# yuanzhi-zhu/DiffPIR

Hardware: AMD Instinct MI355X
Metric: restored images/sec @100 NFE, 256x256 (higher is better)
Workload: dtype f32 (GEMMs as 3 x f16 MFMA on hi/lo-split fp32 operands, fp32 accumulate; exact-fp32-MFMA mode in alt_precision); 1 GPU; configs[1]: ffhq topology 256x256 deblur (61x61 Gaussian PSF), 100 NFE, batch 16/GPU, device Philox noise, hipGraph=on; global_batch=16, nfe=100, collective=none

## Files before the change

diffpir_amd/_lib.py:

```python
from __future__ import annotations

import ctypes as C
import os

_HERE = os.path.dirname(os.path.abspath(__file__))
LIB_PATH = os.environ.get("DIFFPIR_LIB") or os.path.join(_HERE, "csrc", "libdiffpir_hip.so")
ABI_VERSION = 2



class UNetDesc(C.Structure):
    _fields_ = [("image_size", C.c_int32), ("in_channels", C.c_int32), ("model_channels", C.c_int32),
                ("out_channels", C.c_int32), ("num_res_blocks", C.c_int32), ("num_head_channels", C.c_int32),
                ("n_channel_mult", C.c_int32), ("channel_mult", C.c_float * 8),
                ("n_attention_ds", C.c_int32), ("attention_ds", C.c_int32 * 8), ("num_classes", C.c_int32)]


class Tensor(C.Structure):
    _fields_ = [("name", C.c_char_p), ("data", C.c_void_p), ("ndim", C.c_int32), ("shape", C.c_int64 * 4)]


class Step(C.Structure):
    _fields_ = [("t", C.c_int32), ("last", C.c_int32), ("c1", C.c_float), ("c2", C.c_float), ("tau", C.c_float),
                ("sa_t", C.c_float), ("s1m_t", C.c_float), ("sa_p", C.c_float),
# ... 160 lines not shown
    "dpir_unet_flops": (C.c_double, [C.c_void_p, C.c_int, C.c_int]),
    "dpir_unet_flops_class": (C.c_double, [C.c_void_p, C.c_int, C.c_int, C.c_int]),
}

_lib = None


class EngineLibraryError(RuntimeError):
    pass


DEBUG_LIB_PATH = os.path.join(_HERE, "csrc", "libdiffpir_dbg.so")
_dbg = None


def load_debug():
    global _dbg
    if _dbg is not None:
        return _dbg
    load()
    if not os.path.exists(DEBUG_LIB_PATH):
        raise EngineLibraryError(f"{DEBUG_LIB_PATH} not found: `make -C diffpir_amd/csrc` builds it next to the product library")
    d = C.CDLL(DEBUG_LIB_PATH)
    d.dpir_debug_conv_bench.argtypes = [C.c_void_p] + [C.c_int] * 10 + [C.POINTER(C.c_double)]
    d.dpir_debug_conv7_emit_supported.argtypes = [C.c_void_p] + [C.c_int] * 4 + [C.POINTER(C.c_int)]
    d.dpir_debug_victim.argtypes = [C.c_void_p, C.c_int, C.c_int, C.c_int, C.c_longlong, C.c_int, C.POINTER(C.c_ulonglong)]
    d.dpir_debug_victim_alu.argtypes = [C.c_void_p, C.c_int, C.c_int, C.c_int, C.c_int, C.POINTER(C.c_ulonglong)]
    for fn in (d.dpir_debug_victim_fft_pk, d.dpir_debug_victim_fft_nopk):
        fn.argtypes = [C.c_void_p, C.c_int, C.c_int, C.c_int, C.POINTER(C.c_ulonglong)]
    d.dpir_debug_conv7_check.argtypes = [C.c_void_p] + [C.c_int] * 10 + [C.POINTER(C.c_double), C.POINTER(C.c_double), C.POINTER(C.c_ulonglong),
                                                                        C.POINTER(C.c_float), C.POINTER(C.c_int)]
    d.dpir_debug_conv5_layer.argtypes = [C.c_void_p] + [C.c_int] * 7 + [C.c_void_p] * 7 + [C.POINTER(C.c_int)]
    d.dpir_debug_conv5_layer.restype = C.c_int
    d.dpir_debug_conv3_layer.argtypes = [C.c_void_p, C.POINTER(Conv3Desc)]
    d.dpir_debug_conv3_layer.restype = C.c_int
    d.dpir_debug_conv9_layer.argtypes = [C.c_void_p, C.POINTER(Conv9Desc)]
    d.dpir_debug_conv9_layer.restype = C.c_int
    d.dpir_debug_conv11_layer.argtypes = [C.c_void_p, C.POINTER(Conv11Desc)]
    d.dpir_debug_conv11_layer.restype = C.c_int
    d.dpir_debug_conv11_counts.argtypes = [C.POINTER(C.c_longlong), C.POINTER(C.c_longlong)]
    d.dpir_debug_conv11_counts.restype = None
    d.dpir_debug_conv_up_layer.argtypes = [C.c_void_p, C.POINTER(ConvUpDesc)]
    d.dpir_debug_conv_up_layer.restype = C.c_int
    d.dpir_debug_conv_up_counts.argtypes = [C.POINTER(C.c_longlong), C.POINTER(C.c_longlong)]
    d.dpir_debug_conv_up_counts.restype = None
    d.dpir_debug_attention.argtypes = [C.c_void_p, C.POINTER(AttentionDesc)]
    d.dpir_debug_attention.restype = C.c_int
    d.dpir_debug_groupnorm.argtypes = [C.c_void_p, C.POINTER(GroupNormDesc)]
    d.dpir_debug_groupnorm.restype = C.c_int
    for n in ("dpir_debug_conv_bench", "dpir_debug_victim", "dpir_debug_victim_alu", "dpir_debug_victim_fft_pk", "dpir_debug_victim_fft_nopk",
              "dpir_debug_conv7_check"):
        getattr(d, n).restype = C.c_int
    _dbg = d
    return d


def load():
    global _lib
    if _lib is not None:
        return _lib
    if not os.path.exists(LIB_PATH):
        raise EngineLibraryError(
            f"{LIB_PATH} not found: build it with `python -c 'import __graft_entry__ as g; g.build()'` "
            f"or `make -C diffpir_amd/csrc`.  There is no CPU fallback.")
    try:
        import torch
# ... 18 lines not shown
```

diffpir_amd/csrc/dbg_conv.hip:

```cpp
#include "engine.h"
#include "conv6_params.h"
#include "conv9.h"
#include "conv11.h"
#include "conv_up.h"
#include "../../include/diffpir_debug.h"
#include <string.h>
#include <vector>
using namespace dpir;
static int fail(dpir_engine* e, const Status& s) {
    if (e) e->last_error = s.msg;
    return s.code;
}
#define API_TRY(e, expr)                          \
    do {                                          \
        Status _s = (expr);                       \
        if (!_s.ok()) return fail((e), _s);       \
    } while (0)
#define API_HIP(e, expr)                                                                  \
    do {                                                                                  \
        hipError_t _h = (expr);                                                           \
        if (_h != hipSuccess)                                                             \
            return fail((e), Status{DPIR_ERR_HIP, std::string(#expr) + ": " + hipGetErrorString(_h)}); \
    } while (0)

__global__ void dbg_bitdiff_kernel(const float* a, const float* b, size_t n, unsigned long long* out) {
    unsigned long long cnt = 0; unsigned mx = 0;
    for (size_t i = (size_t)blockIdx.x * blockDim.x + threadIdx.x; i < n; i += (size_t)gridDim.x * blockDim.x) {
        const float x = a[i], y = b[i];
        if (__builtin_bit_cast(unsigned, x) != __builtin_bit_cast(unsigned, y)) {
            ++cnt;
            const float d = fabsf(x - y);
            const unsigned u = d == d ? __builtin_bit_cast(unsigned, d) : 0x7fc00000u;
            mx = u > mx ? u : mx;
        }
    }
    if (cnt) { atomicAdd(&out[0], cnt); atomicMax(&out[1], (unsigned long long)mx); }
}
// ... 149 lines not shown
    PendingConv pend;
    API_TRY(e, launch_conv6(e->stream, a6, &k6, &pend));
    if ((S > 1) != (k6 == 3) || (S > 1 && pend.ksplit != S)) return fail(e, Status{DPIR_ERR_INVALID, "conv7 check: the split rule of launch_conv6 changed"});
    API_TRY(e, launch_conv7(e->stream, k, blocks * S, x1 != 0));
    API_HIP(e, hipGetLastError());
    if (S > 1) {
        hipLaunchKernelGGL(dbg_bitdiff_kernel, dim3(2048), dim3(256), 0, e->stream, p6, p7, (size_t)S * no, cmp);
    } else {
        hipLaunchKernelGGL(dbg_bitdiff_kernel, dim3(2048), dim3(256), 0, e->stream, o6, o7, no, cmp);
        hipLaunchKernelGGL(dbg_bitdiff_kernel, dim3(256), dim3(256), 0, e->stream, reinterpret_cast<const float*>(st6), reinterpret_cast<const float*>(st7), nst * 2, cmp);
    }
    unsigned long long h[2] = {0, 0};
    API_HIP(e, hipMemcpyAsync(h, cmp, 16, hipMemcpyDeviceToHost, e->stream));
    API_HIP(e, hipStreamSynchronize(e->stream));
    *mismatches_out = h[0];
    const unsigned mb = (unsigned)h[1];
    *maxdiff_out = __builtin_bit_cast(float, mb);
    hipEvent_t e0, e1, e2;
    API_HIP(e, hipEventCreate(&e0)); API_HIP(e, hipEventCreate(&e1)); API_HIP(e, hipEventCreate(&e2));
    for (int i = 0; i < 3; ++i) { API_TRY(e, launch_conv6(e->stream, a6, &k6, &pend)); API_TRY(e, launch_conv7(e->stream, k, blocks * S, x1 != 0)); }
    API_HIP(e, hipEventRecord(e0, e->stream));
    for (int i = 0; i < iters; ++i) API_TRY(e, launch_conv6(e->stream, a6, &k6, &pend));
    API_HIP(e, hipEventRecord(e1, e->stream));
    for (int i = 0; i < iters; ++i) API_TRY(e, launch_conv7(e->stream, k, blocks * S, x1 != 0));
    API_HIP(e, hipEventRecord(e2, e->stream));
    API_HIP(e, hipEventSynchronize(e2));
    float m6 = 0, m7 = 0;
    API_HIP(e, hipEventElapsedTime(&m6, e0, e1)); API_HIP(e, hipEventElapsedTime(&m7, e1, e2));
    (void)hipEventDestroy(e0); (void)hipEventDestroy(e1); (void)hipEventDestroy(e2);
    *ms6_out = m6 / iters; *ms7_out = m7 / iters;
    return DPIR_OK;
}

int dpir_debug_conv5_layer(dpir_engine* e, int B, int ca, int cb, int Cout, int H, int W, int tile, const float* xa, const float* xb,
                           const float* w, const float* bias, const float* prm, const float* res, float* out, int* path_out) {
    if (!e || !xa || !w || !bias || !out || !path_out || B <= 0 || ca <= 0 || cb < 0 || (cb > 0 && !xb) || Cout <= 0 || tile < 0 || tile > 2) return DPIR_ERR_INVALID;
    if (e->precision == 0) return fail(e, invalid("conv5 layer: the engine is in f32 mode"));
    (void)hipSetDevice(e->device);
    const int C = ca + cb, HW = H * W;
    const size_t na = (size_t)B * ca * HW, nb = (size_t)B * cb * HW, no = (size_t)B * Cout * HW;
    float *dxa = nullptr, *dxb = nullptr, *dbias = nullptr, *dout = nullptr, *dres = nullptr, *dw = nullptr, *partial = nullptr; float4* dprm = nullptr;
    API_TRY(e, e->ws.getT("c5#xa", na, &dxa));
    API_TRY(e, e->ws.getT("c5#xb", nb + 1, &dxb));
    API_TRY(e, e->ws.getT("c5#b", (size_t)round_up(Cout, 64), &dbias));
    API_TRY(e, e->ws.getT("c5#o", no, &dout));
    API_TRY(e, e->ws.getT("c5#res", no, &dres));
    API_TRY(e, e->ws.getT("c5#prm", (size_t)B * C, &dprm));
    API_HIP(e, hipMemcpy(dxa, xa, na * 4, hipMemcpyHostToDevice));
    if (cb) API_HIP(e, hipMemcpy(dxb, xb, nb * 4, hipMemcpyHostToDevice));
    API_HIP(e, hipMemset(dbias, 0, (size_t)round_up(Cout, 64) * 4));
    API_HIP(e, hipMemcpy(dbias, bias, (size_t)Cout * 4, hipMemcpyHostToDevice));
    if (prm) API_HIP(e, hipMemcpy(dprm, prm, (size_t)B * C * 16, hipMemcpyHostToDevice));
    if (res) API_HIP(e, hipMemcpy(dres, res, no * 4, hipMemcpyHostToDevice));
    API_HIP(e, hipMemset(dout, 0xFF, no * 4));
    std::vector<uint16_t> w16v;
    const float w16_scale = pack_weights_f16x3_1x1(w, Cout, C, w16v);
    void* wp = nullptr;
    API_TRY(e, e->ws.get("c5#w16", w16v.size() * 2, &wp));
    API_HIP(e, hipMemcpy(wp, w16v.data(), w16v.size() * 2, hipMemcpyHostToDevice));
    const bool has_prm = prm != nullptr;
    const bool use5 = !(has_prm && C % 16) && (tile != 0 || conv5_supported(B, Cout, H, W, has_prm) || conv5_small_supported(B, ca, cb, Cout, H, W, has_prm));
    Status st;
    if (use5) {
        Conv5Args a5;
        a5.src = CatSrc{dxa, ca, cb ? dxb : nullptr, cb}; a5.prm = has_prm ? dprm : nullptr; a5.w16 = wp; a5.w16_scale = w16_scale;
        a5.bias = dbias; a5.out = dout; a5.res = res ? dres : nullptr; a5.B = B; a5.Cout = Cout; a5.H = H; a5.W = W;
        a5.x1 = e->precision == 2; a5.force_tile = tile;
        *path_out = tile ? tile : (conv5_small_supported(B, ca, cb, Cout, H, W, has_prm) ? 2 : 1);
        st = launch_conv5(e->stream, a5);
    } else {
        const int coutp = round_up(Cout, 64), cinp = round_up(C, 16);
        std::vector<float> packed((size_t)cinp * coutp, 0.f);
        for (int co = 0; co < Cout; ++co)
            for (int ci = 0; ci < C; ++ci) packed[(size_t)ci * coutp + co] = w[(size_t)co * C + ci];
        API_TRY(e, e->ws.getT("c5#w", packed.size(), &dw));
        API_HIP(e, hipMemcpy(dw, packed.data(), packed.size() * 4, hipMemcpyHostToDevice));
        API_TRY(e, e->ws.getT("conv#partial", (size_t)16 * 1024 * 1024, &partial));
        ConvArgs a;
        a.src.a = dxa; a.src.ca = ca; a.src.b = cb ? dxb : nullptr; a.src.cb = cb; a.src.Hs = H; a.src.Ws = W; a.src.mode = 0;
        a.src.prm = has_prm ? dprm : nullptr;
        a.w = dw; a.bias = dbias; a.out = dout; a.res = res ? dres : nullptr; a.res_mode = 0;
        a.B = B; a.Cin = C; a.Cout = Cout; a.CoutP = coutp; a.H = H; a.W = W; a.ks = 1;
        a.partial = partial; a.partial_capacity = (size_t)16 * 1024 * 1024;
        *path_out = 0;
        st = launch_conv(e->stream, a);
    }
    API_TRY(e, st);
    API_HIP(e, hipStreamSynchronize(e->stream));
    API_HIP(e, hipMemcpy(out, dout, no * 4, hipMemcpyDeviceToHost));
    return DPIR_OK;
}

int dpir_debug_conv3_layer(dpir_engine* e, dpir_debug_conv3_desc* d) {
    if (!e || !d) return DPIR_ERR_INVALID;
    d->path_out = -1; d->ksplit_out = 0; d->stat_kind_out = 0;
    const int B = d->B, ca = d->ca, cb = d->cb, Cout = d->Cout, H = d->H, W = d->W, mode = d->mode, C = ca + cb;
    if (!d->xa || !d->w || !d->bias || !d->out || B <= 0 || ca <= 0 || cb < 0 || (cb > 0 && !d->xb) || Cout <= 0 || H <= 0 || W <= 0 || mode < 0 || mode > 2 ||
        d->res_mode < -1 || d->res_mode > 2 || (d->res_mode >= 0 && !d->res) || d->prologue < 0 || d->prologue > 2 ||
        (d->route != 0 && d->route != 6 && d->route != 7 && d->route != 8))
        return fail(e, invalid("conv3 layer: bad descriptor"));
    if (d->prologue == 1 && !d->prm) return fail(e, invalid("conv3 layer: prologue 1 needs the table"));
    if (d->prologue == 2 && (!d->gamma || !d->beta)) return fail(e, invalid("conv3 layer: prologue 2 needs gamma and beta"));
    if (mode == 1 && ((H | W) & 1)) return fail(e, invalid("conv3 layer: a nearest-up source needs an even output size"));
    if (d->res_mode == 1 && ((H | W) & 1)) return fail(e, invalid("conv3 layer: a half-resolution residual needs an even output size"));
    if (d->defer && (!d->split || (d->route != 0 && d->route != 7) || !d->gamma2 || !d->beta2 || !d->w2 || !d->bias2 || !d->out2 || d->Cout2 <= 0))
        return fail(e, invalid("conv3 layer: defer needs split, route 0 or 7 and the second stage's operands"));
    (void)hipSetDevice(e->device);
    const int Hs = mode == 1 ? H / 2 : (mode == 2 ? H * 2 : H), Ws = mode == 1 ? W / 2 : (mode == 2 ? W * 2 : W);
    const size_t HWs = (size_t)Hs * Ws, HW = (size_t)H * W;
    const size_t na = (size_t)B * ca * HWs, nb = (size_t)B * cb * HWs, no = (size_t)B * Cout * HW;
    const size_t nres = d->res_mode == 1 ? no / 4 : (d->res_mode == 2 ? no * 4 : no);
    const int coutp = round_up(Cout, 64);
    float *dxa = nullptr, *dxb = nullptr, *dbias = nullptr, *dout = nullptr, *dres = nullptr, *scale = nullptr; float4* dprm = nullptr;
    API_TRY(e, e->ws.getT("c3#xa", na, &dxa));
    API_TRY(e, e->ws.getT("c3#xb", nb + 1, &dxb));
    API_TRY(e, e->ws.getT("c3#b", (size_t)coutp, &dbias));
    API_TRY(e, e->ws.getT("c3#o", no, &dout));
    API_TRY(e, e->ws.getT("c3#res", nres, &dres));
    API_TRY(e, e->ws.getT("c3#prm", (size_t)B * C, &dprm));
    API_TRY(e, e->ws.getT("c3#scale", (size_t)4, &scale));
    API_HIP(e, hipMemcpy(dxa, d->xa, na * 4, hipMemcpyHostToDevice));
    if (cb) API_HIP(e, hipMemcpy(dxb, d->xb, nb * 4, hipMemcpyHostToDevice));
    API_HIP(e, hipMemset(dbias, 0, (size_t)coutp * 4));
    API_HIP(e, hipMemcpy(dbias, d->bias, (size_t)Cout * 4, hipMemcpyHostToDevice));
// ... 569 lines not shown
```

diffpir_amd/csrc/unet.hip:

```cpp
#include "engine.h"
#include "conv6_params.h"
#include "conv9.h"
#include "conv11.h"
#include "conv_up.h"
#include <unordered_map>
#include <cstdint>
#include <math.h>
#include <string.h>
#include <stdlib.h>

namespace dpir {

Status Workspace::get(const std::string& name, size_t bytes, void** out) {
    auto it = bufs.find(name);
    if (it != bufs.end() && it->second.bytes >= bytes) { *out = it->second.p; return Status{}; }
    if (frozen) return Status{DPIR_ERR_STATE, "workspace allocation of '" + name + "' during graph capture"};
    if (it != bufs.end()) { (void)hipFree(it->second.p); total -= it->second.bytes; bufs.erase(it); }
    void* p = nullptr;
    size_t rb = (bytes + 255) & ~(size_t)255;
    hipError_t err = hipMalloc(&p, rb);
    if (err != hipSuccess) return Status{DPIR_ERR_NOMEM, "hipMalloc(" + std::to_string(rb) + ") for '" + name + "' failed"};
    bufs[name] = DevBuf{p, rb};
    total += rb;
    ++generation;
    *out = p;
    return Status{};
}
void Workspace::release() {
    for (auto& kv : bufs) (void)hipFree(kv.second.p);
    bufs.clear();
    total = 0;
}

namespace {
struct WeightMap {
    std::map<std::string, const dpir_tensor*> m;
// ... 322 lines not shown
                DPIR_TRY(ws.getT(tag + "#gst", (size_t)B * 32, &ga.stats_out));
                if (prm_out) *prm_out = ga.prm_out;
                if (stats_out) *stats_out = ga.stats_out;
            }
            {
                ProfScope ps(&e->prof, PC_ELEM);
                DPIR_TRY(launch_gn_act_small(s, ga));
            }
            if (pending.partial) { fused.erase(pending.out); pending = PendingConv{}; }
            return conv6_on_planes(cw, s16, plane, res, res_mode, out, Ho, Wo, emit);
        }
        DPIR_TRY(resolve());
        float4* prm = nullptr;
        DPIR_TRY(gn(g, in, tag, film_off, true, &prm, stats_out));
        if (prm_out) *prm_out = prm;
        return conv(cw, in, mode, prm, res, res_mode, out, Ho, Wo, emit);
    }

    bool conv9_route(const ConvW& cw, int Ho, int Wo, bool hop) const {
        static const bool on = !(getenv("DPIR_CONV9") && atoi(getenv("DPIR_CONV9")) == 0);
        static const int min_wg = getenv("DPIR_CONV9_MIN_WG") ? atoi(getenv("DPIR_CONV9_MIN_WG")) : kConv9MinWg;
        return on && !grad && e->precision != 0 && cw.w16 && cw.ks == 3 && conv9_supported(B, cw.cin, cw.cout, Ho, Wo, hop) &&
               (long long)B * (cw.cout / 32) >= min_wg;
    }

    bool conv11_route(const ConvW& cw, int Ho, int Wo, bool hop) const {
        static const bool on = !(getenv("DPIR_CONV11") && atoi(getenv("DPIR_CONV11")) == 0);
        static const int split_below = getenv("DPIR_SPLIT_BELOW") ? atoi(getenv("DPIR_SPLIT_BELOW")) : 256;
        if (!on || grad || e->precision != 1 || !cw.w11 || cw.ks != 3 || !conv11_supported(cw.cin, cw.cout, Ho, Wo)) return false;
        const long long wgs = (long long)(Wo / 32) * (Ho / 8) * B * (cw.cout / 128);
        return hop ? wgs >= 384 && conv11_emit_supported(cw.cout, Ho, Wo) : wgs >= split_below;
    }

    Status conv6_on_planes(const ConvW& cw, char* s16, size_t plane, const float* res, int res_mode, float* out, int Ho, int Wo,
                           const Conv6Emit* emit = nullptr) {
        const bool x1 = e->precision == 2;
        Conv6Args a6;
        a6.x1 = x1;
        a6.xhi = s16; a6.xlo = s16 + plane; a6.w16 = cw.w16; a6.w16_scale = cw.w16_scale;
        a6.bias = cw.bias; a6.out = out; a6.res = res; a6.res_mode = res_mode;
        a6.B = B; a6.Cin = cw.cin; a6.Cout = cw.cout; a6.H = Ho; a6.W = Wo;
        a6.partial = partial; a6.partial_capacity = partial_cap;
        const int slots = conv6_stat_slots(Ho, Wo);
        float2* st = nullptr; double2* sp = nullptr;
        if (slots > 0 && cw.cout % 32 == 0) {
            const std::string key = std::to_string(reinterpret_cast<uintptr_t>(out));
            DPIR_TRY(ws.getT("st#" + key, (size_t)B * cw.cout * slots, &st));
            DPIR_TRY(ws.getT("sp#" + key, (size_t)B * cw.cout, &sp));
        }
        a6.stat = st; a6.stat_plane = sp;
        a6.emit = emit;
        if (emit) { a6.stat = nullptr; a6.stat_plane = nullptr; a6.partial = nullptr; a6.partial_capacity = 0; }
        int kind = 0;
        PendingConv pc;
        ProfScope ps(&e->prof, PC_CONV3);
        if (conv9_route(cw, Ho, Wo, emit != nullptr)) {
            Conv9Args a9;
            a9.xhi = s16; a9.xlo = s16 + plane; a9.w16 = cw.w16; a9.w16_scale = cw.w16_scale; a9.bias = cw.bias; a9.out = out;
            a9.res = res; a9.res_mode = res_mode; a9.B = B; a9.Cin = cw.cin; a9.Cout = cw.cout; a9.H = Ho; a9.W = Wo;
            a9.stat_plane = emit ? nullptr : sp; a9.x1 = x1; a9.emit = emit;
            DPIR_TRY(launch_conv9(s, a9));
            if (sp && !emit) fused[out] = FusedStat{nullptr, 0, sp};
            else fused.erase(out);
            return Status{};
        }
        if (conv11_route(cw, Ho, Wo, emit != nullptr)) {
// ... 23 lines not shown
        if (pending.partial && (is_pending(in.a) || is_pending(in.b) || is_pending(res) || !use5)) DPIR_TRY(resolve());
        static const bool use_conv8 = !(getenv("DPIR_CONV8") && atoi(getenv("DPIR_CONV8")) == 0);
        if (use_conv8 && cw.w8 && prm && !grad && !emit && !res && mode == 0 && !in.b && in.H == Ho && in.W == Wo &&
            conv8_supported(B, in.C(), cw.cout, Ho, Wo)) {
            Conv8Args a8;
            a8.x = in.a; a8.prm = prm; a8.w = cw.w8; a8.w_scale = cw.w8_scale; a8.bias = cw.bias; a8.out = out;
            a8.B = B; a8.C = in.C(); a8.Cout = cw.cout; a8.H = Ho; a8.W = Wo; a8.range_ctr = e->range_ctr; a8.x1 = x1;
            fused.erase(out);
            ProfScope ps(&e->prof, PC_CONV3);
            return launch_conv8(s, a8);
        }
        if (cw.w16 && cw.ks == 3 && conv6_supported(Ho, Wo)) {
            int eh = mode == 1 ? Ho / 2 : (mode == 2 ? Ho * 2 : Ho), ew = mode == 1 ? Wo / 2 : (mode == 2 ? Wo * 2 : Wo);
            if (eh != in.H || ew != in.W) return invalid("conv: source resolution does not match mode");
            const int C = in.C(), C8 = 2 * ((C + 15) / 16);
            const size_t plane = (size_t)B * C8 * Ho * Wo * 16;
            if (plane >= ((size_t)1 << 32)) return invalid("conv: split activation plane exceeds the 4 GiB buffer-descriptor range; reduce the batch");
            char* s16 = nullptr;
            DPIR_TRY(ws.getT("act#s16", 2 * plane, &s16));
            {
                ProfScope ps(&e->prof, PC_ELEM);
                DPIR_TRY(launch_act_split(s, CatSrc{in.a, in.ca, in.b, in.cb}, prm, mode, B, Ho, Wo, s16, x1 ? nullptr : s16 + plane, e->range_ctr));
            }
            return conv6_on_planes(cw, s16, plane, res, res_mode, out, Ho, Wo, emit);
        }
        if (emit) return invalid("conv: fused emission was requested for a launch that is not on the f16 3x3 path");
        if (use5) {
            Conv5Args a5;
            a5.src = CatSrc{in.a, in.ca, in.b, in.cb}; a5.prm = prm; a5.w16 = cw.w16; a5.w16_scale = cw.w16_scale;
            a5.bias = cw.bias; a5.out = out; a5.res = res; a5.B = B; a5.Cout = cw.cout; a5.H = Ho; a5.W = Wo;
            a5.range_ctr = e->range_ctr; a5.x1 = x1;
            fused.erase(out);
            ProfScope ps(&e->prof, PC_CONV1);
            return launch_conv5(s, a5);
        }
        fused.erase(out);
        ConvArgs a;
        a.src.a = in.a; a.src.ca = in.ca; a.src.b = in.b; a.src.cb = in.cb; a.src.Hs = in.H; a.src.Ws = in.W;
        a.src.mode = mode; a.src.prm = prm;
        a.w = cw.w; a.bias = cw.bias; a.out = out; a.res = res; a.res_mode = res_mode;
        a.B = B; a.Cin = cw.cin; a.Cout = cw.cout; a.CoutP = cw.coutp; a.H = Ho; a.W = Wo; a.ks = cw.ks;
        a.partial = partial; a.partial_capacity = partial_cap;
        ProfScope ps(&e->prof, cw.ks == 3 ? PC_CONV3 : PC_CONV1);
        return launch_conv(s, a);
    }
    Status gn(const GnW& g, const Act& in, const std::string& tag, int film_off, bool silu, float4** prm_out, float2** stats_out = nullptr) {
        float4* prm = nullptr;
        float2* gst = nullptr;
        if (grad) DPIR_TRY(ws.getT(tag + "#gst", (size_t)B * 32, &gst));
        if (is_pending(in.a) || is_pending(in.b)) DPIR_TRY(resolve());
        DPIR_TRY(ws.getT(tag + "#prm", (size_t)B * g.c, &prm));
        GnStatSrc src[2];
        const float* tp[2] = {in.a, in.b};
        const int tc[2] = {in.ca, in.cb};
        for (int k = 0; k < 2; ++k) {
            src[k].c = tc[k];
            if (!tp[k] || tc[k] == 0) { src[k].c = 0; continue; }
            auto it = fused.find(tp[k]);
            if (it != fused.end()) { src[k].slots = it->second.slots; src[k].nslots = it->second.nslots; src[k].part = it->second.part; continue; }
            double2* part = nullptr;
            DPIR_TRY(ws.getT(tag + "#stats" + std::to_string(k), (size_t)B * tc[k], &part));
            ProfScope ps(&e->prof, PC_GN);
            DPIR_TRY(launch_gn_stats(s, CatSrc{tp[k], tc[k], nullptr, 0}, B, in.H * in.W, part));
            src[k].part = part;
        }
        ProfScope ps(&e->prof, PC_ELEM);
// ... 385 lines not shown
```

include/diffpir_debug.h:

```cpp
#ifndef DIFFPIR_DEBUG_H
#define DIFFPIR_DEBUG_H
#include "diffpir_engine.h"
#ifdef __cplusplus
extern "C" {
#endif
int dpir_debug_conv_bench(dpir_engine* e, int B, int Cin, int Cout, int H, int W, int ks, int mode, int with_prm,
                          int dbg, int iters, double* ms_out);
int dpir_debug_victim(dpir_engine* e, int lds_bytes, int threads, int blocks, long long spin_ticks, int iters, unsigned long long* bad_out);
int dpir_debug_victim_alu(dpir_engine* e, int mode, int blocks, int iters_in_kernel, int launches, unsigned long long* bad_out);
int dpir_debug_victim_fft_pk(dpir_engine* e, int blocks, int iters_in_kernel, int launches, unsigned long long* bad_out);
int dpir_debug_victim_fft_nopk(dpir_engine* e, int blocks, int iters_in_kernel, int launches, unsigned long long* bad_out);
int dpir_debug_conv7_check(dpir_engine* e, int B, int Cin, int Cout, int H, int W, int res_mode, int x1, int split, int scaled, int iters,
                           double* ms6_out, double* ms7_out, unsigned long long* mismatches_out, float* maxdiff_out, int* ksplit_out);
int dpir_debug_conv7_emit_supported(dpir_engine* e, int B, int Cout, int H, int W, int* capacity_out);
int dpir_debug_conv5_layer(dpir_engine* e, int B, int ca, int cb, int Cout, int H, int W, int tile, const float* xa, const float* xb,
                           const float* w, const float* bias, const float* prm, const float* res, float* out, int* path_out);
typedef struct dpir_debug_conv3_desc {
    int32_t B, ca, cb, Cout, H, W, mode, res_mode, scaled, prologue, route, split, defer, Cout2;
    const float *xa, *xb, *w, *bias, *res, *prm, *gamma, *beta, *film, *gamma2, *beta2, *w2, *bias2;
    float* out; double* stat_out; float* out2;
    int32_t stat_kind_out, path_out, ksplit_out, reserved;
} dpir_debug_conv3_desc;
int dpir_debug_conv3_layer(dpir_engine* e, dpir_debug_conv3_desc* d);
typedef struct dpir_debug_conv9_desc {
    int32_t B, Cin, Cout, H, W, res_mode, hop, Cout2;
    const float *x, *w, *bias, *res, *prm, *gamma2, *beta2, *film2, *w2, *bias2;
    float* out; double* stat_out; float* out2;
    int32_t ran_out, iters;
    double ms_out;
} dpir_debug_conv9_desc;
int dpir_debug_conv9_layer(dpir_engine* e, dpir_debug_conv9_desc* d);
typedef struct dpir_debug_conv11_desc {
    int32_t B, Cin, Cout, H, W, res_mode, route, ksplit, hop, Cout2;
    const float *x, *w, *bias, *res, *prm, *gamma2, *beta2, *film2, *w2, *bias2;
    float* out; double* stat_out; float* out2;
    int32_t ran_out, iters;
    double ms_out;
} dpir_debug_conv11_desc;
int dpir_debug_conv11_layer(dpir_engine* e, dpir_debug_conv11_desc* d);
void dpir_debug_conv11_counts(long long* plain, long long* hop);
typedef struct dpir_debug_conv_up_desc {
    int32_t B, Cin, Cout, Hs, Ws, hop, force_hop, Cout2, route, reserved;
    const float *x, *w, *bias, *res, *prm, *gamma2, *beta2, *film2, *w2, *bias2;
    float* out; double* stat_out; float* out2;
    int32_t ran_out, iters;
    double ms_out;
} dpir_debug_conv_up_desc;
int dpir_debug_conv_up_layer(dpir_engine* e, dpir_debug_conv_up_desc* d);
void dpir_debug_conv_up_counts(long long* plain, long long* hop);
// ... 20 lines not shown
```

Baseline: 9.565 images/s.

## Add K-split 1x1 conv kernel with per-wave channel chunks for deep low-pixel layers

Adds a new 1x1 convolution kernel for the f16-split MFMA path. Each of the four waves in a workgroup takes a strided subset of 16-channel input chunks, streams them through a per-wave LDS ring with DMA loads and register-held weights, then sums the partial accumulators through LDS in the epilogue. In the UNet it replaces launch_conv5 for layers with at least 32 input chunks whose grid fits within two resident workgroups per CU, targeting deep, low-resolution 1x1 convs that otherwise underfill the GPU. The cost is an extra LDS reduction and another code path; it can be disabled with an environment variable, and debug timing hooks are added.

```diff
diff --git a/diffpir_amd/_lib.py b/diffpir_amd/_lib.py
--- a/diffpir_amd/_lib.py
+++ b/diffpir_amd/_lib.py
@@ -216,6 +216,10 @@
                                                                         C.POINTER(C.c_float), C.POINTER(C.c_int)]
     d.dpir_debug_conv5_layer.argtypes = [C.c_void_p] + [C.c_int] * 7 + [C.c_void_p] * 7 + [C.POINTER(C.c_int)]
     d.dpir_debug_conv5_layer.restype = C.c_int
+    d.dpir_debug_conv5_layer_time.argtypes = [C.c_void_p] + [C.c_int] * 7 + [C.c_void_p] * 7 + [C.POINTER(C.c_int), C.c_int, C.POINTER(C.c_double)]
+    d.dpir_debug_conv5_layer_time.restype = C.c_int
+    d.dpir_debug_conv5k_count.argtypes = []
+    d.dpir_debug_conv5k_count.restype = C.c_longlong
     d.dpir_debug_conv3_layer.argtypes = [C.c_void_p, C.POINTER(Conv3Desc)]
     d.dpir_debug_conv3_layer.restype = C.c_int
     d.dpir_debug_conv9_layer.argtypes = [C.c_void_p, C.POINTER(Conv9Desc)]
diff --git a/diffpir_amd/csrc/conv5k.h b/diffpir_amd/csrc/conv5k.h
--- /dev/null
+++ b/diffpir_amd/csrc/conv5k.h
@@ -0,0 +1,12 @@
+#pragma once
+#include "common.h"
+namespace dpir {
+
+const char* conv5k_refusal(int B, int ca, int cb, int Cout, int H, int W, bool has_prm);
+Status launch_conv5k(hipStream_t s, const Conv5Args& a);
+long long conv5k_workgroups(int B, int Cout, int H, int W);
+int conv5k_resident_workgroups();
+constexpr int kConv5kMinChunks = 32;
+long long conv5k_launch_count();
+
+}
diff --git a/diffpir_amd/csrc/conv5k.hip b/diffpir_amd/csrc/conv5k.hip
--- /dev/null
+++ b/diffpir_amd/csrc/conv5k.hip
@@ -0,0 +1,340 @@
+#include "common.h"
+#include "lds_dma.h"
+#include "conv5k.h"
+#include <type_traits>
+#include <atomic>
+
+namespace dpir {
+
+typedef float floatx16 __attribute__((ext_vector_type(16)));
+typedef _Float16 half8 __attribute__((ext_vector_type(8)));
+
+struct Conv5kK {
+    const float* sa; const float* sb; int ca, cb;
+    unsigned bytes_a, bytes_b, bytes_w, bytes_prm;
+    const float4* prm;
+    const char* w16; const float* bias; float* out; const float* res;
+    int B, Cout, HW;
+    int n_chunks, n_co_blocks;
+    int n_wblocks;
+    int n_tiles, pair_xcd;
+    int total_px;
+    float out_scale;
+    unsigned long long* range_ctr;
+};
+
+template <int I, int N, class F>
+__device__ __forceinline__ void static_for5k(F&& f) {
+    if constexpr (I < N) {
+        f(std::integral_constant<int, I>{});
+        static_for5k<I + 1, N>(f);
+    }
+}
+
+__device__ __forceinline__ float gn_apply5k(float v, const float4 m, bool silu) {
+    float t = (v - m.x) * m.y + m.z;
+    if (silu) t = t * __builtin_amdgcn_rcpf(1.0f + __builtin_amdgcn_exp2f(t * -1.4426950408889634f));
+    return t;
+}
+
+typedef unsigned u32x4k __attribute__((ext_vector_type(4)));
+template <int IMM>
+__device__ __forceinline__ half8 load_a5k(unsigned voff, u32x4k rsrc, unsigned soff) {
+    half8 r;
+    asm volatile("buffer_load_dwordx4 %0, %1, %2, %3 offen offset:%4" : "=v"(r) : "v"(voff), "s"(rsrc), "s"(soff), "n"(IMM) : "memory");
+    return r;
+}
+
+constexpr int kC5kTpx = 128;
+constexpr int kC5kRedStride = kC5kTpx + 4;
+constexpr int kC5kRedBytes = 4 * 32 * kC5kRedStride * 4;
+static_assert(2 * (kC5kRedBytes + 256) <= 160 * 1024, "two workgroups per CU");
+
+template <bool HAS_PRM, bool X1>
+__device__ __forceinline__ bool conv5k_chunk(const float* __restrict__ xs, const float4* __restrict__ ps, const int (&pimg)[4], int l31, bool silu,
+                                             const half8 (&ah)[2], const half8 (&al)[2], floatx16 (&acc)[2][4]) {
+    bool bad = false;
+#pragma unroll
+    for (int jp = 0; jp < 4; jp += 2) {
+        half8 bh[2], bl[2];
+#pragma unroll
+        for (int jj2 = 0; jj2 < 2; ++jj2) {
+            const int j = jp + jj2;
+            float v[8];
+#pragma unroll
+            for (int jj = 0; jj < 8; ++jj) v[jj] = xs[jj * kC5kTpx + j * 32 + l31];
+            if (HAS_PRM) {
+#pragma unroll
+                for (int jj = 0; jj < 8; ++jj) v[jj] = gn_apply5k(v[jj], ps[pimg[j] * 16 + jj], silu);
+            }
+#pragma unroll
+            for (int jj = 0; jj < 8; ++jj) {
+                bad |= !(fabsf(v[jj]) <= 65000.f);
+                float x = fminf(fmaxf(v[jj], -65000.f), 65000.f);
+                _Float16 hh = (_Float16)x;
+                bh[jj2][jj] = hh;
+                if (!X1) bl[jj2][jj] = (_Float16)(x - (float)hh);
+            }
+        }
+        if (!X1) {
+#pragma unroll
+            for (int i = 0; i < 2; ++i)
+#pragma unroll
+                for (int jj2 = 0; jj2 < 2; ++jj2)
+                    acc[i][jp + jj2] = __builtin_amdgcn_mfma_f32_32x32x16_f16(al[i], bh[jj2], acc[i][jp + jj2], 0, 0, 0);
+#pragma unroll
+            for (int i = 0; i < 2; ++i)
+#pragma unroll
+                for (int jj2 = 0; jj2 < 2; ++jj2)
+                    acc[i][jp + jj2] = __builtin_amdgcn_mfma_f32_32x32x16_f16(ah[i], bl[jj2], acc[i][jp + jj2], 0, 0, 0);
+        }
+#pragma unroll
+        for (int i = 0; i < 2; ++i)
+#pragma unroll
+            for (int jj2 = 0; jj2 < 2; ++jj2)
+                acc[i][jp + jj2] = __builtin_amdgcn_mfma_f32_32x32x16_f16(ah[i], bh[jj2], acc[i][jp + jj2], 0, 0, 0);
+    }
+    return bad;
+}
+
+template <bool HAS_PRM, bool X1, int NBUF>
+__global__ __launch_bounds__(256, NBUF == 2 ? 2 : 1) void conv5k_kernel(Conv5kK p) {
+#if defined(__HIP_DEVICE_COMPILE__)
+    static_assert(NBUF >= 2 && NBUF <= 4, "ring depths the counted wait's immediate covers");
+    constexpr int TCO = 64, TPX = kC5kTpx;
+    constexpr int XBYTES = 16 * TPX * 4;
+    constexpr int PBYTES = HAS_PRM ? 1024 : 0;
+    constexpr int WB = XBYTES + PBYTES;
+    constexpr int WAVE_LDS = NBUF * WB;
+    constexpr int MAIN = 4 * WAVE_LDS > kC5kRedBytes ? 4 * WAVE_LDS : kC5kRedBytes;
+    constexpr int NX = XBYTES / 1024;
+    constexpr int NA = X1 ? 2 : 4;
+    constexpr int NG = NX + (HAS_PRM ? 1 : 0) + NA;
+    __shared__ __attribute__((aligned(16))) char smem5k[MAIN + 256];
+    float* bias_sh = reinterpret_cast<float*>(smem5k + MAIN);
+
+    const int tid = threadIdx.x;
+    const int lane = tid & 63;
+    const int wave = __builtin_amdgcn_readfirstlane(tid >> 6);
+    const int l31 = lane & 31;
+    const int half = lane >> 5;
+    const int bid = blockIdx.x;
+    int co_blk, tile;
+    if (p.pair_xcd) {
+        const int t = bid >> 3;
+        co_blk = t % p.n_co_blocks;
+        tile = 8 * (t / p.n_co_blocks) + (bid & 7);
+        if (tile >= p.n_tiles) return;
+    } else {
+        co_blk = bid % p.n_co_blocks;
+        tile = bid / p.n_co_blocks;
+    }
+    const int px0 = tile * TPX;
+    const int C = p.ca + p.cb;
+    const int HW = p.HW;
+    const int total_px = p.total_px;
+    const int n_tile = px0 / HW;
+
+    const __amdgpu_buffer_rsrc_t rs_a = rsrc_uniform(p.sa, p.bytes_a);
+    const __amdgpu_buffer_rsrc_t rs_b = rsrc_uniform(p.sb ? p.sb : p.sa, p.sb ? p.bytes_b : 0u);
+    u32x4k rw;
+    {
+        const unsigned long long wa = reinterpret_cast<unsigned long long>(p.w16);
+        rw[0] = __builtin_amdgcn_readfirstlane((unsigned)wa); rw[1] = __builtin_amdgcn_readfirstlane((unsigned)(wa >> 32));
+        rw[2] = __builtin_amdgcn_readfirstlane(p.bytes_w); rw[3] = 0x00020000u;
+    }
+    const __amdgpu_buffer_rsrc_t rs_p = rsrc_uniform(HAS_PRM ? (const void*)p.prm : (const void*)p.w16, HAS_PRM ? p.bytes_prm : 0u);
+    const int lr = lane >> 5;
+    const int gq = px0 + 4 * (lane & 31);
+    const bool q_ok = gq < total_px;
+    const int qn = q_ok ? gq / HW : 0;
+    const int qp = q_ok ? gq - qn * HW : 0;
+    const unsigned voffA = q_ok ? (unsigned)(((size_t)qn * p.ca * HW + (size_t)lr * HW + qp) * 4) : kOutOfRange;
+    const unsigned voffB = q_ok ? (unsigned)(((size_t)qn * p.cb * HW + (size_t)lr * HW + qp) * 4) : kOutOfRange;
+    const unsigned voffP = (HAS_PRM && n_tile + (lane >> 4) < p.B) ? (unsigned)(((size_t)(n_tile + (lane >> 4)) * C + (lane & 15)) * 16) : kOutOfRange;
+    const unsigned voffW = (unsigned)(half * 128 + (co_blk & 1) * 64 + l31) * 16u;
+
+    char* const wlds = smem5k + wave * WAVE_LDS;
+    half8 a_h[NBUF][2], a_l[NBUF][2];
+    auto issue = [&](int chunk, auto slot_c) __attribute__((always_inline)) {
+        constexpr int slot = decltype(slot_c)::value;
+        char* buf = wlds + slot * WB;
+        const bool live = chunk < p.n_chunks;
+#pragma unroll
+        for (int u = 0; u < NX; ++u) {
+            const int c = chunk * 16 + u * 2;
+            char* dst = buf + u * 1024;
+            if (c < p.ca) BLDS6(rs_a, dst, c + lr < p.ca ? voffA : kOutOfRange, (unsigned)c * (unsigned)HW * 4u);
+            else BLDS6(rs_b, dst, c + lr < C ? voffB : kOutOfRange, live ? (unsigned)(c - p.ca) * (unsigned)HW * 4u : 0u);
+        }
+        if constexpr (HAS_PRM) BLDS6(rs_p, buf + XBYTES, live ? voffP : kOutOfRange, live ? (unsigned)chunk * 256u : 0u);
+        const unsigned wsoff = live ? (unsigned)(chunk * p.n_wblocks + (co_blk >> 1)) * 8192u : 0u;
+        const unsigned vw = live ? voffW : kOutOfRange - 8192u;
+        a_h[slot][0] = load_a5k<0>(vw, rw, wsoff);
+        if (!X1) a_l[slot][0] = load_a5k<0>(vw + 4096u, rw, wsoff);
+        a_h[slot][1] = load_a5k<512>(vw, rw, wsoff);
+        if (!X1) a_l[slot][1] = load_a5k<512>(vw + 4096u, rw, wsoff);
+    };
+
+    int pimg[4];
+#pragma unroll
+    for (int j = 0; j < 4; ++j) {
+        const int g = px0 + j * 32 + l31;
+        pimg[j] = (g < total_px ? g / HW : n_tile) - n_tile;
+    }
+
+    floatx16 acc[2][4];
+#pragma unroll
+    for (int i = 0; i < 2; ++i)
+#pragma unroll
+        for (int j = 0; j < 4; ++j)
+#pragma unroll
+            for (int r = 0; r < 16; ++r) acc[i][j][r] = 0.f;
+
+    bool bad = false;
+    bool silu = false;
+    if (HAS_PRM) silu = __builtin_amdgcn_readfirstlane(p.prm[0].w != 0.f ? 1 : 0) != 0;
+    if (tid < TCO) bias_sh[tid] = co_blk * TCO + tid < p.Cout ? p.bias[co_blk * TCO + tid] : 0.f;
+
+    const int nk = wave < p.n_chunks ? (p.n_chunks - wave + 3) >> 2 : 0;
+    __builtin_amdgcn_sched_barrier(0);
+    static_for5k<0, NBUF - 1>([&](auto s_c) __attribute__((always_inline)) { issue(wave + 4 * decltype(s_c)::value, s_c); });
+    for (int k0 = 0; k0 < nk; k0 += NBUF) {
+        static_for5k<0, NBUF>([&](auto s_c) __attribute__((always_inline)) {
+            constexpr int s = decltype(s_c)::value, sp = (s + NBUF - 1) % NBUF;
+            __builtin_amdgcn_sched_barrier(0);
+            __builtin_amdgcn_s_waitcnt(15 | (7 << 4) | (0 << 8) | (3 << 14));
+            issue(wave + 4 * (k0 + s + NBUF - 1), std::integral_constant<int, sp>{});
+            __builtin_amdgcn_sched_barrier(0);
+            wait_vmcnt<(NBUF - 1) * NG>();
+            __builtin_amdgcn_sched_barrier(0);
+            const char* buf = wlds + s * WB;
+            if (k0 + s < nk)
+                bad |= conv5k_chunk<HAS_PRM, X1>(reinterpret_cast<const float*>(buf) + (8 * half) * TPX,
+                                                 reinterpret_cast<const float4*>(buf + XBYTES) + 8 * half, pimg, l31, silu, a_h[s], a_l[s], acc);
+        });
+    }
+    wait_vmcnt<0>();
+
+    {
+        const unsigned long long m = __ballot(bad);
+        if (m != 0ull && p.range_ctr && lane == __builtin_ctzll(m)) atomicAdd(p.range_ctr, (unsigned long long)__builtin_popcountll(m));
+    }
+
+    float* const red = reinterpret_cast<float*>(smem5k);
+    const int row_l = tid >> 5, c4 = tid & 31;
+    const int g4 = px0 + 4 * c4;
+    const bool ok4 = g4 < total_px;
+    const int n4 = ok4 ? g4 / HW : 0;
+    const size_t base4 = (size_t)n4 * p.Cout * HW + (size_t)(g4 - n4 * HW);
+    const int co0 = co_blk * TCO;
+    const float osc = p.out_scale;
+#pragma unroll
+    for (int i = 0; i < 2; ++i) {
+        __syncthreads();
+#pragma unroll
+        for (int j = 0; j < 4; ++j)
+#pragma unroll
+            for (int r = 0; r < 16; ++r)
+                red[(wave * 32 + (r & 3) + 8 * (r >> 2) + 4 * half) * kC5kRedStride + j * 32 + l31] = acc[i][j][r];
+        __syncthreads();
+        float4 rr[4];
+        if (p.res) {
+#pragma unroll
+            for (int sw = 0; sw < 4; ++sw) {
+                const int co = co0 + i * 32 + sw * 8 + row_l;
+                rr[sw] = (ok4 && co < p.Cout) ? *reinterpret_cast<const float4*>(p.res + base4 + (size_t)co * HW) : make_float4(0.f, 0.f, 0.f, 0.f);
+            }
+            wait_vmcnt<0>();
+        }
+#pragma unroll
+        for (int sw = 0; sw < 4; ++sw) {
+            const int row = sw * 8 + row_l;
+            const int co = co0 + i * 32 + row;
+            float4 a4 = *reinterpret_cast<const float4*>(red + row * kC5kRedStride + 4 * c4);
+#pragma unroll
+            for (int w = 1; w < 4; ++w) {
+                const float4 t = *reinterpret_cast<const float4*>(red + (w * 32 + row) * kC5kRedStride + 4 * c4);
+                a4 = make_float4(a4.x + t.x, a4.y + t.y, a4.z + t.z, a4.w + t.w);
+            }
+            const float bz = bias_sh[i * 32 + row];
+            if (ok4 && co < p.Cout) {
+                float4 v = make_float4(a4.x * osc + bz, a4.y * osc + bz, a4.z * osc + bz, a4.w * osc + bz);
+                if (p.res) v = make_float4(rr[sw].x + v.x, rr[sw].y + v.y, rr[sw].z + v.z, rr[sw].w + v.w);
+                *reinterpret_cast<float4*>(p.out + base4 + (size_t)co * HW) = v;
+            }
+        }
+    }
+#endif
+}
+
+const char* conv5k_refusal(int B, int ca, int cb, int Cout, int H, int W, bool has_prm) {
+    if (B <= 0 || ca <= 0 || cb < 0 || Cout <= 0 || H <= 0 || W <= 0) return "conv5k: empty launch";
+    const long long HW = (long long)H * W, px = (long long)B * HW;
+    if (HW % 4) return "conv5k: float4 stores need H * W % 4 == 0";
+    if (has_prm && HW % 64) return "conv5k: the GroupNorm variant stages the table rows of at most 4 images per tile (H * W % 64 == 0)";
+    if (has_prm && (ca + cb) % 16) return "conv5k: the GroupNorm variant needs a multiple of 16 input channels";
+    if (cb > 0 && ca % 4) return "conv5k: a DMA instruction covers two channel rows; the concat boundary must be a multiple of 4";
+    if (px >= (1ll << 31) - 256) return "conv5k: more than 2^31 pixels in the batch";
+    const unsigned long long chunks = (unsigned long long)(ca + cb + 15) / 16, wblocks = (unsigned long long)(Cout + 127) / 128;
+    if ((unsigned long long)px * ca * 4 >= (1ull << 32) || (unsigned long long)px * cb * 4 >= (1ull << 32) || chunks * wblocks * 8192 >= (1ull << 31) ||
+        (unsigned long long)B * (ca + cb) * 16 >= (1ull << 32))
+        return "conv5k: an input tensor exceeds the 4 GiB buffer-descriptor range; reduce the batch";
+    return nullptr;
+}
+
+static std::atomic<long long> g_conv5k_launches{0};
+long long conv5k_launch_count() { return g_conv5k_launches.load(); }
+
+static int conv5k_cus() {
+    static std::atomic<int> cached[16];
+    int dev = 0, cus = 0;
+    if (hipGetDevice(&dev) != hipSuccess) return 0;
+    std::atomic<int>* slot = (dev >= 0 && dev < 16) ? &cached[dev] : nullptr;
+    if (slot && slot->load() > 0) return slot->load();
+    if (hipDeviceGetAttribute(&cus, hipDeviceAttributeMultiprocessorCount, dev) != hipSuccess) return 0;
+    if (slot) slot->store(cus);
+    return cus;
+}
+
+long long conv5k_workgroups(int B, int Cout, int H, int W) { return (((long long)B * H * W + kC5kTpx - 1) / kC5kTpx) * ((Cout + 63) / 64); }
+int conv5k_resident_workgroups() { return 2 * conv5k_cus(); }
+
+template <bool HAS_PRM, bool X1>
+static void launch5k(hipStream_t s, const Conv5kK& k, unsigned blocks) {
+    hipLaunchKernelGGL((conv5k_kernel<HAS_PRM, X1, 2>), dim3(blocks), dim3(256), 0, s, k);
+}
+
+Status launch_conv5k(hipStream_t s, const Conv5Args& a) {
+    const int ca = a.src.ca, cb = a.src.b ? a.src.cb : 0;
+    const bool has_prm = a.prm != nullptr;
+    if (const char* why = conv5k_refusal(a.B, ca, cb, a.Cout, a.H, a.W, has_prm)) return Status{DPIR_ERR_UNSUPPORTED, why};
+    if (a.emit_hi || a.emit_prm || a.out_scale_dev) return invalid("conv5k: plain forward launches only (no emitted planes, no device output scale)");
+    if (!a.src.a || !a.w16 || !a.bias || !a.out) return invalid("conv5k: input, f16 weight pack, bias and output are required");
+    Conv5kK k;
+    k.sa = a.src.a; k.sb = cb ? a.src.b : nullptr; k.ca = ca; k.cb = cb; k.prm = a.prm;
+    k.w16 = reinterpret_cast<const char*>(a.w16); k.bias = a.bias; k.out = a.out; k.res = a.res;
+    k.B = a.B; k.Cout = a.Cout; k.HW = a.H * a.W;
+    const int C = ca + cb;
+    k.n_chunks = (C + 15) / 16;
+    k.n_co_blocks = (a.Cout + 63) / 64;
+    k.n_wblocks = (a.Cout + 127) / 128;
+    const long long total_px = (long long)a.B * a.H * a.W;
+    k.total_px = (int)total_px;
+    k.bytes_a = (unsigned)((unsigned long long)total_px * ca * 4); k.bytes_b = (unsigned)((unsigned long long)total_px * cb * 4);
+    k.bytes_w = (unsigned)((unsigned long long)k.n_chunks * k.n_wblocks * 8192); k.bytes_prm = (unsigned)((unsigned long long)a.B * C * 16);
+    k.out_scale = 1.0f / a.w16_scale;
+    k.range_ctr = a.range_ctr;
+    k.n_tiles = (int)((total_px + kC5kTpx - 1) / kC5kTpx);
+    static const bool pair_env = !(getenv("DPIR_CONV5_PAIR") && atoi(getenv("DPIR_CONV5_PAIR")) == 0);
+    k.pair_xcd = pair_env && k.n_co_blocks > 1 ? 1 : 0;
+    const unsigned blocks = k.pair_xcd ? (unsigned)((k.n_tiles + 7) / 8 * 8 * k.n_co_blocks) : (unsigned)(k.n_tiles * k.n_co_blocks);
+    if (a.x1) { if (has_prm) launch5k<true, true>(s, k, blocks); else launch5k<false, true>(s, k, blocks); }
+    else if (has_prm) launch5k<true, false>(s, k, blocks);
+    else launch5k<false, false>(s, k, blocks);
+    DPIR_HIP(hipGetLastError());
+    g_conv5k_launches.fetch_add(1);
+    return Status{};
+}
+
+}
diff --git a/diffpir_amd/csrc/dbg_conv.hip b/diffpir_amd/csrc/dbg_conv.hip
--- a/diffpir_amd/csrc/dbg_conv.hip
+++ b/diffpir_amd/csrc/dbg_conv.hip
@@ -3,6 +3,7 @@
 #include "conv9.h"
 #include "conv11.h"
 #include "conv_up.h"
+#include "conv5k.h"
 #include "../../include/diffpir_debug.h"
 #include <string.h>
 #include <vector>
@@ -218,10 +219,14 @@
     return DPIR_OK;
 }
 
-int dpir_debug_conv5_layer(dpir_engine* e, int B, int ca, int cb, int Cout, int H, int W, int tile, const float* xa, const float* xb,
-                           const float* w, const float* bias, const float* prm, const float* res, float* out, int* path_out) {
-    if (!e || !xa || !w || !bias || !out || !path_out || B <= 0 || ca <= 0 || cb < 0 || (cb > 0 && !xb) || Cout <= 0 || tile < 0 || tile > 2) return DPIR_ERR_INVALID;
+static int conv5_layer_run(dpir_engine* e, int B, int ca, int cb, int Cout, int H, int W, int tile, const float* xa, const float* xb,
+                           const float* w, const float* bias, const float* prm, const float* res, float* out, int* path_out, int iters, double* us_out) {
+    if (!e || !xa || !w || !bias || !out || !path_out || B <= 0 || ca <= 0 || cb < 0 || (cb > 0 && !xb) || Cout <= 0 || tile < 0 || tile > 3) return DPIR_ERR_INVALID;
     if (e->precision == 0) return fail(e, invalid("conv5 layer: the engine is in f32 mode"));
+    if (tile == 3) {
+        if (e->grad_enabled) return fail(e, Status{DPIR_ERR_UNSUPPORTED, "conv5k layer: a gradient-mode engine keeps launch_conv5's route"});
+        if (const char* why = conv5k_refusal(B, ca, cb, Cout, H, W, prm != nullptr)) return fail(e, Status{DPIR_ERR_UNSUPPORTED, why});
+    }
     (void)hipSetDevice(e->device);
     const int C = ca + cb, HW = H * W;
     const size_t na = (size_t)B * ca * HW, nb = (size_t)B * cb * HW, no = (size_t)B * Cout * HW;
@@ -247,11 +252,18 @@
     const bool has_prm = prm != nullptr;
     const bool use5 = !(has_prm && C % 16) && (tile != 0 || conv5_supported(B, Cout, H, W, has_prm) || conv5_small_supported(B, ca, cb, Cout, H, W, has_prm));
     Status st;
-    if (use5) {
-        Conv5Args a5;
+    Conv5Args a5;
+    if (tile == 3 || use5) {
         a5.src = CatSrc{dxa, ca, cb ? dxb : nullptr, cb}; a5.prm = has_prm ? dprm : nullptr; a5.w16 = wp; a5.w16_scale = w16_scale;
         a5.bias = dbias; a5.out = dout; a5.res = res ? dres : nullptr; a5.B = B; a5.Cout = Cout; a5.H = H; a5.W = W;
-        a5.x1 = e->precision == 2; a5.force_tile = tile;
+        a5.x1 = e->precision == 2;
+    }
+    if (tile == 3) {
+        a5.range_ctr = e->range_ctr;
+        *path_out = 3;
+        st = launch_conv5k(e->stream, a5);
+    } else if (use5) {
+        a5.force_tile = tile;
         *path_out = tile ? tile : (conv5_small_supported(B, ca, cb, Cout, H, W, has_prm) ? 2 : 1);
         st = launch_conv5(e->stream, a5);
     } else {
@@ -274,8 +286,33 @@
     API_TRY(e, st);
     API_HIP(e, hipStreamSynchronize(e->stream));
     API_HIP(e, hipMemcpy(out, dout, no * 4, hipMemcpyDeviceToHost));
+    if (iters > 0 && us_out) {
+        if (*path_out == 0) return fail(e, invalid("conv5 layer: only the conv5 tiles and conv5k are timed"));
+        hipEvent_t e0, e1;
+        API_HIP(e, hipEventCreate(&e0)); API_HIP(e, hipEventCreate(&e1));
+        API_HIP(e, hipEventRecord(e0, e->stream));
+        for (int it = 0; it < iters && st.ok(); ++it) st = *path_out == 3 ? launch_conv5k(e->stream, a5) : launch_conv5(e->stream, a5);
+        API_HIP(e, hipEventRecord(e1, e->stream));
+        API_HIP(e, hipStreamSynchronize(e->stream));
+        float ms = 0.f;
+        API_HIP(e, hipEventElapsedTime(&ms, e0, e1));
+        (void)hipEventDestroy(e0); (void)hipEventDestroy(e1);
+        API_TRY(e, st);
+        *us_out = 1e3 * ms / iters;
+    }
     return DPIR_OK;
 }
+
+int dpir_debug_conv5_layer(dpir_engine* e, int B, int ca, int cb, int Cout, int H, int W, int tile, const float* xa, const float* xb,
+                           const float* w, const float* bias, const float* prm, const float* res, float* out, int* path_out) {
+    return conv5_layer_run(e, B, ca, cb, Cout, H, W, tile, xa, xb, w, bias, prm, res, out, path_out, 0, nullptr);
+}
+int dpir_debug_conv5_layer_time(dpir_engine* e, int B, int ca, int cb, int Cout, int H, int W, int tile, const float* xa, const float* xb,
+                                const float* w, const float* bias, const float* prm, const float* res, float* out, int* path_out, int iters, double* us_out) {
+    if (iters <= 0 || !us_out) return DPIR_ERR_INVALID;
+    return conv5_layer_run(e, B, ca, cb, Cout, H, W, tile, xa, xb, w, bias, prm, res, out, path_out, iters, us_out);
+}
+long long dpir_debug_conv5k_count(void) { return conv5k_launch_count(); }
 
 int dpir_debug_conv3_layer(dpir_engine* e, dpir_debug_conv3_desc* d) {
     if (!e || !d) return DPIR_ERR_INVALID;
diff --git a/diffpir_amd/csrc/unet.hip b/diffpir_amd/csrc/unet.hip
--- a/diffpir_amd/csrc/unet.hip
+++ b/diffpir_amd/csrc/unet.hip
@@ -2,6 +2,7 @@
 #include "conv6_params.h"
 #include "conv9.h"
 #include "conv11.h"
+#include "conv5k.h"
 #include "conv_up.h"
 #include <unordered_map>
 #include <cstdint>
@@ -390,6 +391,15 @@
         return hop ? wgs >= 384 && conv11_emit_supported(cw.cout, Ho, Wo) : wgs >= split_below;
     }
 
+    bool conv5k_route(const Act& in, int Cout, int Ho, int Wo, bool has_prm) const {
+        static const bool on = !(getenv("DPIR_CONV5K") && atoi(getenv("DPIR_CONV5K")) == 0);
+        static const int min_chunks = getenv("DPIR_CONV5K_MIN_CHUNKS") ? atoi(getenv("DPIR_CONV5K_MIN_CHUNKS")) : kConv5kMinChunks;
+        const int ca = in.ca, cb = in.b ? in.cb : 0;
+        return on && !grad && e->precision != 0 && conv5_small_supported(B, ca, cb, Cout, Ho, Wo, has_prm) &&
+               conv5k_refusal(B, ca, cb, Cout, Ho, Wo, has_prm) == nullptr && (ca + cb + 15) / 16 >= min_chunks &&
+               conv5k_workgroups(B, Cout, Ho, Wo) <= conv5k_resident_workgroups();
+    }
+
     Status conv6_on_planes(const ConvW& cw, char* s16, size_t plane, const float* res, int res_mode, float* out, int Ho, int Wo,
                            const Conv6Emit* emit = nullptr) {
         const bool x1 = e->precision == 2;
@@ -479,6 +489,7 @@
             a5.range_ctr = e->range_ctr; a5.x1 = x1;
             fused.erase(out);
             ProfScope ps(&e->prof, PC_CONV1);
+            if (conv5k_route(in, cw.cout, Ho, Wo, prm != nullptr)) return launch_conv5k(s, a5);
             return launch_conv5(s, a5);
         }
         fused.erase(out);
diff --git a/include/diffpir_debug.h b/include/diffpir_debug.h
--- a/include/diffpir_debug.h
+++ b/include/diffpir_debug.h
@@ -15,6 +15,10 @@
 int dpir_debug_conv7_emit_supported(dpir_engine* e, int B, int Cout, int H, int W, int* capacity_out);
 int dpir_debug_conv5_layer(dpir_engine* e, int B, int ca, int cb, int Cout, int H, int W, int tile, const float* xa, const float* xb,
                            const float* w, const float* bias, const float* prm, const float* res, float* out, int* path_out);
+int dpir_debug_conv5_layer_time(dpir_engine* e, int B, int ca, int cb, int Cout, int H, int W, int tile, const float* xa, const float* xb,
+                                const float* w, const float* bias, const float* prm, const float* res, float* out, int* path_out, int iters,
+                                double* us_out);
+long long dpir_debug_conv5k_count(void);
 typedef struct dpir_debug_conv3_desc {
     int32_t B, ca, cb, Cout, H, W, mode, res_mode, scaled, prologue, route, split, defer, Cout2;
     const float *xa, *xb, *w, *bias, *res, *prm, *gamma, *beta, *film, *gamma2, *beta2, *w2, *bias2;
```

Result: no change. 9.584 images/s, median of 6 (+0.2%).
